# OmerMersin/video-stab

Measured on AMD Instinct MI355X. Metric: stabilized frames/sec @1080p (whole job; warp-stage HBM GB/s in roofline), higher is better.
Workload: dtype u8

## Files before the change

include/vs_stab.h:

```cpp
#ifndef VS_STAB_H
#define VS_STAB_H

#include <stddef.h>
#include <stdint.h>

#ifdef __cplusplus
extern "C" {
#endif

#define VS_STAB_ABI_VERSION 2

typedef enum vs_status {
    VS_OK = 0,
    VS_ERR_INVALID_ARG = 1,
    VS_ERR_NO_DEVICE = 2,
    VS_ERR_HIP = 3,
    VS_ERR_UNSUPPORTED = 4,
    VS_ERR_SIZE_CHANGED = 5,
    VS_ERR_CAPACITY = 6
} vs_status;

typedef enum vs_pixfmt {
    VS_FMT_BGR8 = 0,
    VS_FMT_NV12 = 1,
// ... 268 lines not shown
    int32_t push, idx, n_seen, has_M;
    float   M[12];
    double  Minv[12];
} vs_traj_release;
int vs_op_trajectory(const vs_params_c* params, int n_streams, const double* const* models, const int32_t* const* kinds,
                     const int32_t* n_push, int form, const int32_t* steps, int n_steps, vs_debug_frame* const* dbg_out,
                     int32_t* n_dbg, vs_traj_release* const* rel_out, int32_t* n_rel);
int vs_op_resize_gray(const void* d_src, size_t src_stride, int sw, int sh, int fmt,
                      void* d_dst, size_t dst_stride, int dw, int dh, void* stream);
int vs_op_pyr_down(const void* d_src, size_t src_stride, int sw, int sh,
                   void* d_dst, size_t dst_stride, void* stream);
int vs_op_scharr(const void* d_src, size_t src_stride, int w, int h,
                 void* d_dst , void* stream);
int vs_op_pyr_level(const void* d_src, size_t src_stride, size_t src_frame_bytes, int w, int h, void* d_der ,
                    void* d_next, size_t next_stride, size_t next_frame_bytes, int items, void* stream);
int vs_op_pyr_lk(const void* d_prev, const void* d_next, size_t stride, int w, int h,
                 const float* d_prev_pts, int n, float* d_next_pts,
                 uint8_t* d_status, float* d_err,
                 int win, int max_level, int max_iters, double eps, void* stream);
int vs_op_gftt(const void* d_gray, size_t stride, int w, int h, int max_corners,
               double quality, double min_distance, int block_size,
               float* d_pts, int32_t* d_count, float* d_eig, void* stream);
int vs_op_estimate_affine_partial2d(const float* d_from, const float* d_to, int n,
                                    double thr, int max_iters, double* d_model,
                                    uint8_t* d_inliers, int32_t* d_info, void* stream);

void vs_roll_params_default(vs_roll_params_c* p);
int vs_roll_create(const vs_roll_params_c* params, int device, vs_roll** out);
void vs_roll_destroy(vs_roll* r);
const char* vs_roll_last_error(const vs_roll* r);
// ... 140 lines not shown
```

video-stab_amd/csrc/batch_schedule.cpp:

```cpp
#include <cstring>
#include <new>

#include "stab_internal.h"

using namespace vsd;

struct vs_batch {
    int device = 0, S = 0, B = 0, cap = 0;
    bool own = false;
    std::vector<vs_stab*> m;
    vs_stab* ref = nullptr;
    std::string err;
    FirstFailure failure;
    hipStream_t st = nullptr, st_pre = nullptr, st_det = nullptr, st_up = nullptr;
    bool allocated = false;
    uint8_t* h_tables = nullptr;
    size_t h_set_bytes = 0, ho_pairs = 0, ho_lk = 0, ho_rs = 0, ho_tail = 0, ho_gf = 0, ho_seg = 0;
    uint8_t* d_all = nullptr;
    uint8_t *d_lk[2] = {nullptr, nullptr}, *d_rs[2] = {nullptr, nullptr}, *d_tail[2] = {nullptr, nullptr}, *d_seg[2] = {nullptr, nullptr}, *d_gf = nullptr;
    uint8_t* d_tin[2] = {nullptr, nullptr};
    ImgPair* d_pairs[2] = {nullptr, nullptr};
    size_t up_bytes = 0;
    int pre_rel_step = -1;
    double* d_MinvB[2] = {nullptr, nullptr};
// ... 304 lines not shown
    if (k >= 2) VS_OBJ_HIP(g, hipStreamWaitEvent(g->st_up, g->blk_event(k - 2), 0));
    VS_OBJ_HIP(g, hipMemcpyAsync(d_pairs, g->host_set(k).base, g->up_bytes, hipMemcpyHostToDevice, g->st_up));
    VS_OBJ_HIP(g, hipEventRecord(g->ev_up[dset], g->st_up));
    VS_OBJ_HIP(g, hipStreamWaitEvent(pre, g->ev_up[dset], 0));
    {
        StageScope t(g->ref, VS_STAGE_GRAY, pre);
        const int gfmt = s0->pf->gray_source;
        const int n_a = (P.ndet > 0 && P.ndet < n) ? P.ndet : n;
        VS_OBJ_TRY(g, launch_resize_gray_batch(d_pairs, n_a, s0->src_pitch, s0->w, s0->h, gfmt, s0->aw, s0->aw, s0->ah, P.aligned, pre));
        VS_OBJ_HIP(g, hipEventRecord(g->ev_bgray, pre));
        if (n_a < n)
            VS_OBJ_TRY(g, launch_resize_gray_batch(d_pairs + n_a, n - n_a, s0->src_pitch, s0->w, s0->h, gfmt, s0->aw, s0->aw, s0->ah, P.aligned, pre));
    }
    {
        StageScope t(g->ref, VS_STAGE_PYRAMID, pre);
        for (int l = 0; l < s0->levels; l++)
            VS_OBJ_TRY(g, launch_pyr_level_batch(nullptr, d_pairs + (size_t)(l + 1) * n, n, s0->lw[l], s0->lw[l], s0->lh[l], s0->lw[l + 1], pre));
    }
    if (!g->ready.valid) VS_OBJ_HIP(g, hipEventRecord(g->ev_bpre, pre));
    return VS_OK;
}

int step_issue_det(vs_batch* g, const StepPlan& P) {
    const vs_stab* s0 = g->ref;
    const int k = P.k, ndet = P.ndet;
    hipStream_t sd = g->st_det;
    g->det_valid(k) = ndet > 0;
    if (ndet == 0) return VS_OK;
    VS_OBJ_HIP(g, hipMemcpyAsync(g->d_gf, g->host_set(k).gf, gftt_item_bytes() * ndet, hipMemcpyHostToDevice, sd));
    if (k >= 2) VS_OBJ_HIP(g, hipStreamWaitEvent(sd, g->blk_event(k - 2), 0));
    VS_OBJ_TRY(g, launch_gftt_batch(g->d_gf, ndet, s0->aw, s0->ah, 3, sd, 1));
// ... 272 lines not shown
```

video-stab_amd/csrc/k_gftt.hip:

```cpp
#include <cstdio>
#include <cstdlib>

#include <cstring>

#include "vs_common.h"

namespace vsd {
namespace {

constexpr int TW = 64, TH = 16, NT = 256;
constexpr int MAX_BS = 7;

constexpr int SORT_CAP = 8192;
constexpr int CELLS_MAX = 2560;
constexpr int SLOTS = 4;
constexpr int ACC_MAX = 4096;
constexpr int SEL_NT = 256;
constexpr int NMS_ROWS = 8;

__device__ __forceinline__ uint32_t order_key(float v) {
    uint32_t b = __float_as_uint(v);
    return (b & 0x80000000u) ? ~b : (b | 0x80000000u);
}
__device__ __forceinline__ float key_to_float(uint32_t k) {
    uint32_t b = (k & 0x80000000u) ? (k & 0x7FFFFFFFu) : ~k;
    return __uint_as_float(b);
}

template <int BS>
__device__ __forceinline__ void min_eigen_tile(const uint8_t* __restrict__ gray, size_t stride, int w,
                                               int h, int bs_arg, float f1, float* __restrict__ eig,
                                               uint32_t* __restrict__ max_key) {
    constexpr int BSM = BS ? BS : MAX_BS;
    __shared__ uint8_t g[TH + BSM - 1 + 2][TW + BSM - 1 + 2 + 2];
    __shared__ float cxx[TH + BSM - 1][TW + BSM - 1 + 1], cxy[TH + BSM - 1][TW + BSM - 1 + 1], cyy[TH + BSM - 1][TW + BSM - 1 + 1];
    __shared__ uint32_t smax[NT / 64];
    const int bs = BS ? BS : bs_arg;
    const int tid = threadIdx.x;
    const int x0 = blockIdx.x * TW, y0 = blockIdx.y * TH;
    const int anchor = bs / 2, hi = bs - 1 - anchor;
    const int gx0 = x0 - anchor - 1, gy0 = y0 - anchor - 1;
    const int GW = TW + bs - 1 + 2, GH = TH + bs - 1 + 2;
    const int CW = TW + bs - 1, CH = TH + bs - 1;
    const float f0 = 2.f * f1;
    const bool interior = gx0 >= 0 && gy0 >= 0 && gx0 + GW <= w && gy0 + GH <= h;
    if (interior) {
        constexpr int NG = ((TW + BSM - 1 + 2) * (TH + BSM - 1 + 2) + NT - 1) / NT;
// ... 58 lines not shown
            const uint32_t k = order_key(e);
            kmax = k > kmax ? k : kmax;
        }
    }
#pragma unroll
    for (int off = 32; off >= 1; off >>= 1) {
        const uint32_t o = __shfl_xor(kmax, off, 64);
        kmax = o > kmax ? o : kmax;
    }
    if ((tid & 63) == 0) smax[tid >> 6] = kmax;
    __syncthreads();
    if (tid == 0) {
        uint32_t m = smax[0];
        for (int i = 1; i < NT / 64; i++) m = smax[i] > m ? smax[i] : m;
        atomicMax(max_key, m);
    }
}

template <int BS>
__global__ __launch_bounds__(NT) void min_eigen_kernel(const uint8_t* __restrict__ gray, size_t stride, int w,
                                                       int h, int bs, float f1, float* __restrict__ eig,
                                                       uint32_t* __restrict__ max_key) {
    min_eigen_tile<BS>(gray, stride, w, h, bs, f1, eig, max_key);
}

__device__ __forceinline__ void nms_row(const float* __restrict__ eig, int w, int h, double quality,
                                        const uint32_t* __restrict__ max_key,
                                        unsigned long long* __restrict__ cand, int cap,
                                        int32_t* __restrict__ counters) {
    const int x = blockIdx.x * blockDim.x + threadIdx.x;
    const float maxv = key_to_float(*max_key);
    const float thr = (float)((double)maxv * quality);
    const int lane = threadIdx.x & 63;
    float centre[NMS_ROWS];
    {
        const int xc = min(max(x, 0), w - 1);
#pragma unroll
        for (int k = 0; k < NMS_ROWS; k++) centre[k] = eig[(size_t)min((int)blockIdx.y * NMS_ROWS + k, h - 1) * w + xc];
    }
#pragma unroll
    for (int k = 0; k < NMS_ROWS; k++) {
    const int y = blockIdx.y * NMS_ROWS + k;
    if (y >= h) break;
    bool is_cand = false;
    float v = 0.f;
    if (x >= 1 && x < w - 1 && y >= 1 && y < h - 1) {
        const float* r = eig + (size_t)y * w + x;
        v = centre[k] > thr ? centre[k] : 0.f;
// ... 11 lines not shown
        }
    }
    const unsigned long long mask = __ballot(is_cand);
    if (!mask) continue;
    int base = 0;
    if (lane == __ffsll((long long)mask) - 1) base = atomicAdd(&counters[0], __popcll(mask));
    base = __builtin_amdgcn_readlane(base, __ffsll((long long)mask) - 1);
    if (!is_cand) continue;
    const int pos = base + __popcll(mask & ((1ull << lane) - 1ull));
    if (pos < cap) cand[pos] = ((unsigned long long)order_key(v) << 32) | (uint32_t)(y * w + x);
    else counters[2] = 1;
    }
}

__global__ __launch_bounds__(NT) void nms_kernel(const float* __restrict__ eig, int w, int h, double quality,
                                                 const uint32_t* __restrict__ max_key,
                                                 unsigned long long* __restrict__ cand, int cap,
                                                 int32_t* __restrict__ counters) {
    nms_row(eig, w, h, quality, max_key, cand, cap, counters);
}

struct SelArgs {
    const unsigned long long* cand;
    int32_t* counters;
    int cap, w, h, max_corners;
    int min_dist2_i;
    int use_dist;
    int cell, gw, gh;
    float* out_pts;
    int32_t* out_count;
};

template <int E>
__device__ __forceinline__ void bitonic_sort_desc(unsigned long long* keys, int tid) {
// ... 226 lines not shown
        a.counters[3] = s_nacc;
        if (s_overflow) a.counters[2] = 2;
    }
}

__global__ __launch_bounds__(SEL_NT) void select_kernel(SelArgs a) { select_corners(a); }

struct GfttItem {
    const uint8_t* gray;
    size_t stride;
    int w, h, bs;
    float f1;
    double quality;
    float* eig;
    int32_t* counters;
    SelArgs sel;
};

__global__ __launch_bounds__(64) void gftt_zero_batch_kernel(const GfttItem* __restrict__ table) {
    if (threadIdx.x < 16) table[blockIdx.x].counters[threadIdx.x] = 0;
}
template <int BS>
__global__ __launch_bounds__(NT) void min_eigen_batch_kernel(const GfttItem* __restrict__ table) {
    const GfttItem& it = table[blockIdx.z];
    min_eigen_tile<BS>(it.gray, it.stride, it.w, it.h, it.bs, it.f1, it.eig, (uint32_t*)&it.counters[1]);
}
__global__ __launch_bounds__(NT) void nms_batch_kernel(const GfttItem* __restrict__ table) {
    const GfttItem& it = table[blockIdx.z];
    nms_row(it.eig, it.w, it.h, it.quality, (const uint32_t*)&it.counters[1], (unsigned long long*)it.sel.cand, it.sel.cap,
            it.counters);
}
__global__ __launch_bounds__(SEL_NT) void select_batch_kernel(const GfttItem* __restrict__ table) {
    select_corners(table[blockIdx.x].sel);
}

bool gftt_bad_args(const uint8_t* d_gray, const float* d_pts, const int32_t* d_count, int w, int h, int max_corners,
                   int block_size, const GfttWork& wk) {
    return !d_gray || !d_pts || !d_count || w < 3 || h < 3 || w > 65535 || h > 65535 || max_corners <= 0 ||
           max_corners > ACC_MAX || block_size < 1 || block_size > MAX_BS || !wk.eig || !wk.cand || !wk.counters ||
           wk.cap <= 0;
}

void fill_sel_args(SelArgs& a, int w, int h, int max_corners, double min_distance, const GfttWork& wk, float* d_pts,
                   int32_t* d_count) {
    a.cand = (const unsigned long long*)wk.cand;
    a.counters = wk.counters;
    a.cap = wk.cap; a.w = w; a.h = h; a.max_corners = max_corners;
    a.use_dist = min_distance >= 1 ? 1 : 0;
    a.min_dist2_i = (int)std::ceil(std::min(min_distance * min_distance, 2.0e9));
    a.cell = a.use_dist ? (int)lrint(min_distance) : 1;
    a.gw = (w + a.cell - 1) / a.cell;
    a.gh = (h + a.cell - 1) / a.cell;
    a.out_pts = d_pts; a.out_count = d_count;
}
// ... 2 lines not shown

size_t gftt_item_bytes() { return sizeof(GfttItem); }

int gftt_fill_item(void* host_item, const uint8_t* d_gray, size_t stride, int w, int h, int max_corners, double quality,
                   double min_distance, int block_size, const GfttWork& wk, float* d_pts, int32_t* d_count) {
    if (!host_item || gftt_bad_args(d_gray, d_pts, d_count, w, h, max_corners, block_size, wk)) {
        set_last_error("gftt: invalid argument (1 <= blockSize <= 7, 0 < maxCorners <= 4096)");
        return VS_ERR_INVALID_ARG;
    }
    GfttItem& it = *static_cast<GfttItem*>(host_item);
    memset(&it, 0, sizeof it);
    it.gray = d_gray; it.stride = stride; it.w = w; it.h = h; it.bs = block_size;
    double scale = (double)(1 << 2) * block_size * 255.0;
    it.f1 = (float)(1.0 / scale);
    it.quality = quality;
    it.eig = wk.eig; it.counters = wk.counters;
    fill_sel_args(it.sel, w, h, max_corners, min_distance, wk, d_pts, d_count);
    return VS_OK;
}

int launch_gftt_batch(const void* d_table, int items, int w, int h, int block_size, hipStream_t st, int what) {
    if (!d_table || items < 1 || items > 65535 || w < 3 || h < 3 || block_size < 1 || block_size > MAX_BS || what < 0 || what > 5) { set_last_error("gftt_batch: invalid argument"); return VS_ERR_INVALID_ARG; }
    const GfttItem* t = static_cast<const GfttItem*>(d_table);
    if (what == 0 || what == 1) hipLaunchKernelGGL(gftt_zero_batch_kernel, dim3(items), dim3(64), 0, st, t);
    if (what == 0 || what == 2 || what == 4) {
        const dim3 eg((w + TW - 1) / TW, (h + TH - 1) / TH, items);
        if (block_size == 3) hipLaunchKernelGGL(min_eigen_batch_kernel<3>, eg, dim3(NT), 0, st, t);
        else hipLaunchKernelGGL(min_eigen_batch_kernel<0>, eg, dim3(NT), 0, st, t);
    }
    if (what == 0 || what == 2 || what == 5)
        hipLaunchKernelGGL(nms_batch_kernel, dim3((w + NT - 1) / NT, (h + NMS_ROWS - 1) / NMS_ROWS, items), dim3(NT), 0, st, t);
    if (what == 0 || what == 3) hipLaunchKernelGGL(select_batch_kernel, dim3(items), dim3(SEL_NT), 0, st, t);
    VS_HIP_TRY(hipGetLastError());
    return VS_OK;
}

size_t gftt_work_bytes(int w, int h, int cap) {
    return (size_t)w * h * 4 + (size_t)cap * 8 + 64 + 256;
}

void gftt_work_carve(void* base, int w, int h, int cap, GfttWork* out) {
    uint8_t* p = (uint8_t*)base;
    out->eig = (float*)p;
    p += ((size_t)w * h * 4 + 63) & ~(size_t)63;
    out->cand = (uint64_t*)p;
    p += (size_t)cap * 8;
    out->counters = (int32_t*)p;
    out->cap = cap;
}

int launch_gftt(const uint8_t* d_gray, size_t stride, int w, int h, int max_corners, double quality,
                double min_distance, int block_size, const GfttWork& wk, float* d_pts,
                int32_t* d_count, hipStream_t st) {
    if (gftt_bad_args(d_gray, d_pts, d_count, w, h, max_corners, block_size, wk)) {
        set_last_error("gftt: invalid argument (1 <= blockSize <= 7, 0 < maxCorners <= 4096)");
        return VS_ERR_INVALID_ARG;
    }
    VS_HIP_TRY(hipMemsetAsync(wk.counters, 0, 64, st));
    double scale = (double)(1 << 2) * block_size * 255.0;
    scale = 1.0 / scale;
    const float f1 = (float)scale;
    dim3 g1((w + TW - 1) / TW, (h + TH - 1) / TH);
    if (block_size == 3)
        hipLaunchKernelGGL(min_eigen_kernel<3>, g1, dim3(NT), 0, st, d_gray, stride, w, h, block_size, f1, wk.eig, (uint32_t*)&wk.counters[1]);
    else
        hipLaunchKernelGGL(min_eigen_kernel<0>, g1, dim3(NT), 0, st, d_gray, stride, w, h, block_size, f1, wk.eig, (uint32_t*)&wk.counters[1]);
    dim3 g2((w + NT - 1) / NT, (h + NMS_ROWS - 1) / NMS_ROWS);
    hipLaunchKernelGGL(nms_kernel, g2, dim3(NT), 0, st, wk.eig, w, h, quality, (const uint32_t*)&wk.counters[1],
                       (unsigned long long*)wk.cand, wk.cap, wk.counters);
    SelArgs a;
    fill_sel_args(a, w, h, max_corners, min_distance, wk, d_pts, d_count);
    hipLaunchKernelGGL(select_kernel, dim3(1), dim3(SEL_NT), 0, st, a);
    VS_HIP_TRY(hipGetLastError());
    return VS_OK;
}

int run_gftt_op(const uint8_t* d_gray, size_t stride, int w, int h, int max_corners, double quality,
                double min_distance, int block_size, float* d_pts, int32_t* d_count, float* d_eig,
                hipStream_t st) {
    if (w <= 0 || h <= 0) { set_last_error("gftt: invalid size"); return VS_ERR_INVALID_ARG; }
    const int cap = w * h / 4 + 64;
    void* scratch = nullptr;
    VS_HIP_TRY(hipMalloc(&scratch, gftt_work_bytes(w, h, cap)));
// ... 15 lines not shown
```

video-stab_amd/csrc/k_pyr.hip:

```cpp
#include "vs_common.h"

namespace vsd {
namespace {

constexpr int NT = 256;
constexpr int RPB = 4;

__global__ __launch_bounds__(NT) void pyr_down_kernel(const uint8_t* __restrict__ src_, size_t sstride,
                                                      int sw, int sh, uint8_t* __restrict__ dst_,
                                                      size_t dstride, int dw, int dh) {
    const uint8_t* __restrict__ src = src_;
    uint8_t* __restrict__ dst = dst_;
    const int x = blockIdx.x * blockDim.x + threadIdx.x;
    if (x >= dw) return;
    int xi[5];
#pragma unroll
    for (int k = 0; k < 5; k++) xi[k] = reflect101(2 * x + k - 2, sw);
    for (int y = blockIdx.y * RPB; y < min((int)(blockIdx.y + 1) * RPB, dh); y++) {
        int col[5];
#pragma unroll
        for (int j = 0; j < 5; j++) {
            const uint8_t* s = src + (size_t)reflect101(2 * y + j - 2, sh) * sstride;
            col[j] = s[xi[2]] * 6 + (s[xi[1]] + s[xi[3]]) * 4 + s[xi[0]] + s[xi[4]];
        }
// ... 17 lines not shown
    const int a_p = (r0[xp] + r2[xp]) * 3 + r1[xp] * 10;
    const int b_m = r2[xm] - r0[xm];
    const int b_c = r2[x] - r0[x];
    const int b_p = r2[xp] - r0[xp];
    short2 o;
    o.x = (short)(a_p - a_m);
    o.y = (short)((b_p + b_m) * 3 + b_c * 10);
    *reinterpret_cast<short2*>(dst + ((size_t)y * w + x) * 2) = o;
    }
}

constexpr int FT_W = 64, FT_H = 16;
constexpr int FT_PITCH = 72;
constexpr int FT_ROWS = FT_H + 4;

template <bool DER, bool DOWN>
__global__ __launch_bounds__(NT) void pyr_level_kernel(const ImgPair* __restrict__ sch, const ImgPair* __restrict__ pyr, size_t sstride,
                                                       int w, int h, size_t dstride, int dw, int dh) {
    static_assert(DER || DOWN, "a level launch produces something");
    __shared__ __attribute__((aligned(16))) uint8_t tile[FT_ROWS * FT_PITCH];
    const uint8_t* __restrict__ src = static_cast<const uint8_t*>((DER ? sch : pyr)[blockIdx.z].src);
    const int tid = threadIdx.x;
    const int x0 = blockIdx.x * FT_W, y0 = blockIdx.y * FT_H;
    const bool inside = x0 >= 4 && y0 >= 2 && x0 + FT_W + 4 <= w && y0 + FT_H + 2 <= h && (sstride & 3) == 0 && ((uintptr_t)src & 3) == 0;
    if (inside) {
        constexpr int ND = (FT_ROWS * (FT_PITCH / 4) + NT - 1) / NT;
        uint32_t v[ND];
#pragma unroll
        for (int k = 0; k < ND; k++) {
            const int i = min(tid + NT * k, FT_ROWS * (FT_PITCH / 4) - 1);
// ... 45 lines not shown
                const int dx = a[k + 2] - a[k], dy = (b[k + 2] + b[k]) * 3 + b[k + 1] * 10;
                o[k] = ((uint32_t)dx & 0xFFFFu) | ((uint32_t)dy << 16);
            }
            int16_t* d = der + ((size_t)y * w + x) * 2;
            if (x + 3 < w && (((uintptr_t)d) & 15) == 0) {
                *reinterpret_cast<uint4*>(d) = make_uint4(o[0], o[1], o[2], o[3]);
            } else {
                for (int k = 0; k < 4 && x + k < w; k++) reinterpret_cast<uint32_t*>(d)[k] = o[k];
            }
        }
    }
    if (DOWN) {
        uint8_t* __restrict__ dst = static_cast<uint8_t*>(pyr[blockIdx.z].dst);
        const int xo = (x0 >> 1) + (tid & 31), yo = (y0 >> 1) + (tid >> 5);
        if (xo < dw && yo < dh) {
            const int o = 2 * (tid & 31) + 2, sh = o & 3;
            const uint32_t* q = T + 2 * (tid >> 5) * (FT_PITCH / 4) + (o >> 2);
            int col[5];
#pragma unroll
            for (int j = 0; j < 5; j++) {
                const uint32_t lo = q[j * (FT_PITCH / 4)], hi = q[j * (FT_PITCH / 4) + 1];
                const uint32_t four = __builtin_amdgcn_alignbyte(hi, lo, sh);
                const uint32_t fifth = (hi >> (8 * sh)) & 255u;
                col[j] = (int)__builtin_amdgcn_udot4(four, 0x04060401u, fifth, false);
            }
            dst[(size_t)yo * dstride + xo] = (uint8_t)((col[2] * 6 + (col[1] + col[3]) * 4 + col[0] + col[4] + 128) >> 8);
        }
    }
}

}

int launch_pyr_level_batch(const ImgPair* d_scharr_pairs, const ImgPair* d_pyr_pairs, int items, size_t sstride, int w, int h,
                           size_t dstride, hipStream_t st) {
    if ((!d_scharr_pairs && !d_pyr_pairs) || items < 1 || items > 65535 || w <= 0 || h <= 0 || h > 65535) {
        set_last_error("pyr_level_batch: invalid argument");
        return VS_ERR_INVALID_ARG;
    }
    const int dw = (w + 1) / 2, dh = (h + 1) / 2;
    dim3 grid((w + FT_W - 1) / FT_W, (h + FT_H - 1) / FT_H, items);
    if (!d_scharr_pairs)
        hipLaunchKernelGGL((pyr_level_kernel<false, true>), grid, dim3(NT), 0, st, d_scharr_pairs, d_pyr_pairs, sstride, w, h, dstride, dw, dh);
    else if (d_pyr_pairs)
        hipLaunchKernelGGL((pyr_level_kernel<true, true>), grid, dim3(NT), 0, st, d_scharr_pairs, d_pyr_pairs, sstride, w, h, dstride, dw, dh);
    else hipLaunchKernelGGL((pyr_level_kernel<true, false>), grid, dim3(NT), 0, st, d_scharr_pairs, d_pyr_pairs, sstride, w, h, dstride, dw, dh);
    VS_HIP_TRY(hipGetLastError());
    return VS_OK;
}

int launch_pyr_down(const uint8_t* d_src, size_t sstride, int sw, int sh, uint8_t* d_dst,
                    size_t dstride, hipStream_t st) {
    if (!d_src || !d_dst || sw <= 0 || sh <= 0 || sh > 131070) {
        set_last_error("pyr_down: invalid argument");
        return VS_ERR_INVALID_ARG;
    }
    const int dw = (sw + 1) / 2, dh = (sh + 1) / 2;
    dim3 grid((dw + NT - 1) / NT, (dh + RPB - 1) / RPB);
    hipLaunchKernelGGL(pyr_down_kernel, grid, dim3(NT), 0, st, d_src, sstride, sw, sh, d_dst, dstride, dw, dh);
    VS_HIP_TRY(hipGetLastError());
    return VS_OK;
}

int launch_scharr(const uint8_t* d_src, size_t sstride, int w, int h, int16_t* d_dst, hipStream_t st) {
    if (!d_src || !d_dst || w <= 0 || h <= 0 || h > 65535) {
// ... 11 lines not shown
```

video-stab_amd/csrc/vs_api.cpp:

```cpp
#include <cmath>
#include <cstring>
#include <mutex>
#include <vector>

#include "launchers.h"
#include "vs_common.h"

namespace vsd {

static thread_local std::string g_last_error;
void set_last_error(const std::string& msg) { g_last_error = msg; }
const char* get_last_error() { return g_last_error.c_str(); }

int ensure_device() {
    int n = 0;
    hipError_t e = hipGetDeviceCount(&n);
    if (e != hipSuccess || n <= 0) {
        set_last_error(std::string("no HIP device: ") + (e != hipSuccess ? hipGetErrorString(e) : "count is 0") +
                       " (libvideo-stab has no CPU fallback)");
        return VS_ERR_NO_DEVICE;
    }
    return VS_OK;
}

// ... 305 lines not shown
        const uint8_t* s = (const uint8_t*)d_src + (size_t)i * src_frame_bytes;
        t[i] = ImgPair{s, (uint8_t*)d_der + (size_t)i * w * h * 4};
        t[items + i] = ImgPair{s, d_next ? (uint8_t*)d_next + (size_t)i * next_frame_bytes : nullptr};
    }
    ImgPair* d_t = nullptr;
    VS_HIP_TRY(hipMalloc((void**)&d_t, sizeof(ImgPair) * t.size()));
    hipStream_t st = (hipStream_t)stream;
    int rc = VS_OK;
    if (hipMemcpyAsync(d_t, t.data(), sizeof(ImgPair) * t.size(), hipMemcpyHostToDevice, st) != hipSuccess) rc = VS_ERR_HIP;
    if (rc == VS_OK) rc = launch_pyr_level_batch(d_t, d_next ? d_t + items : nullptr, items, src_stride, w, h, next_stride, st);
    (void)hipStreamSynchronize(st);
    (void)hipFree(d_t);
    return rc;
}

int vs_op_pyr_lk(const void* d_prev, const void* d_next, size_t stride, int w, int h,
                 const float* d_prev_pts, int n, float* d_next_pts, uint8_t* d_status, float* d_err,
                 int win, int max_level, int max_iters, double eps, void* stream) {
    VS_TRY(ensure_device());
    return run_pyr_lk_op((const uint8_t*)d_prev, (const uint8_t*)d_next, stride, w, h, d_prev_pts, n,
                         d_next_pts, d_status, d_err, win, max_level, max_iters, eps,
                         (hipStream_t)stream);
}

int vs_op_gftt(const void* d_gray, size_t stride, int w, int h, int max_corners, double quality,
               double min_distance, int block_size, float* d_pts, int32_t* d_count, float* d_eig,
               void* stream) {
    VS_TRY(ensure_device());
    return run_gftt_op((const uint8_t*)d_gray, stride, w, h, max_corners, quality, min_distance,
                       block_size, d_pts, d_count, d_eig, (hipStream_t)stream);
// ... 12 lines not shown
```

video-stab_amd/csrc/vs_common.h:

```cpp
#ifndef VS_COMMON_H
#define VS_COMMON_H

#include <hip/hip_runtime.h>
#include <cstdlib>
#include <stdint.h>
#include <cfloat>
#include <cmath>
#include <string>
#include <utility>

#include "../../include/vs_stab.h"

namespace vsd {

void set_last_error(const std::string& msg);
const char* get_last_error();

inline int hip_fail(hipError_t e, const char* expr) {
    set_last_error(std::string(expr) + ": " + hipGetErrorString(e));
    return (e == hipErrorNoDevice || e == hipErrorInvalidDevice || e == hipErrorInsufficientDriver || e == hipErrorNoBinaryForGpu)
               ? VS_ERR_NO_DEVICE
               : VS_ERR_HIP;
}

// ... 113 lines not shown
    int32_t sw, sh, dw, dh, cn, border;
    double m[6];
    int32_t sb = 1;
};
constexpr int WARP_JOBS_MAX = 24;
int launch_warp_jobs(const WarpJob* jobs, int n, hipStream_t st);
bool scale_job_staged(const WarpJob& j);
int launch_scale_jobs(const WarpJob* jobs, int n, int path, hipStream_t st);
int launch_resize_gray(const uint8_t* d_src, size_t sstride, int sw, int sh, int fmt,
                       uint8_t* d_dst, size_t dstride, int dw, int dh, hipStream_t st);
struct ImgPair { const void* src; void* dst; };
int launch_resize_gray_batch(const ImgPair* d_pairs, int items, size_t sstride, int sw, int sh, int fmt, size_t dstride,
                             int dw, int dh, int aligned, hipStream_t st);
int launch_pyr_level_batch(const ImgPair* d_scharr_pairs, const ImgPair* d_pyr_pairs, int items, size_t sstride, int w, int h,
                           size_t dstride, hipStream_t st);
int launch_pyr_down(const uint8_t* d_src, size_t sstride, int sw, int sh, uint8_t* d_dst,
                    size_t dstride, hipStream_t st);
int launch_scharr(const uint8_t* d_src, size_t sstride, int w, int h, int16_t* d_dst,
                  hipStream_t st);

struct LKLevel {
    const uint8_t* prev;
    const uint8_t* next;
    int w, h;
    size_t stride;
};
int launch_pyr_lk(const LKLevel* levels, int max_level, const float* d_prev_pts, int n,
                  const int32_t* d_n, float* d_next_pts, uint8_t* d_status, float* d_err, int win,
                  int max_iters, double eps, hipStream_t st);

struct GfttWork {
    float* eig;
    uint64_t* cand;
    int32_t* counters;
    int cap;
};
size_t gftt_work_bytes(int w, int h, int cap);
void gftt_work_carve(void* base, int w, int h, int cap, GfttWork* out);
int launch_gftt(const uint8_t* d_gray, size_t stride, int w, int h, int max_corners,
                double quality, double min_distance, int block_size, const GfttWork& wk,
                float* d_pts, int32_t* d_count, hipStream_t st);

}
#endif
```

video-stab_amd/vsamd/capi.py:

```python
import collections
import ctypes as C
import os

import numpy as np

PKG_DIR = os.path.dirname(os.path.dirname(os.path.abspath(__file__)))
LIB_PATH = os.path.join(PKG_DIR, "csrc", "libvideo-stab.so")

u8p = C.POINTER(C.c_uint8)
f32p = C.POINTER(C.c_float)
f64p = C.POINTER(C.c_double)
i32p = C.POINTER(C.c_int32)

PixFmt = collections.namedtuple("PixFmt", "fmt name text kind cn sample_bytes bits sx sy gray_source border_modes")
KIND_INTERLEAVED, KIND_LUMA_UV, KIND_THREE_PLANES = range(3)
PIXFMTS = (
    PixFmt(0, "BGR8", "BGR8", KIND_INTERLEAVED, 3, 1, 8, 0, 0, 0, True),
    PixFmt(1, "NV12", "NV12", KIND_LUMA_UV, 1, 1, 8, 1, 1, 2, False),
    PixFmt(2, "GRAY8", "GRAY8", KIND_INTERLEAVED, 1, 1, 8, 0, 0, 2, False),
    PixFmt(3, "BGRA8", "BGRA8", KIND_INTERLEAVED, 4, 1, 8, 0, 0, 3, True),
    PixFmt(4, "RGBA8", "RGBA8", KIND_INTERLEAVED, 4, 1, 8, 0, 0, 4, True),
    PixFmt(5, "RGB8", "RGB8", KIND_INTERLEAVED, 3, 1, 8, 0, 0, 5, True),
    PixFmt(6, "P010", "P010", KIND_LUMA_UV, 2, 2, 10, 1, 1, 6, False),
    PixFmt(7, "I420", "I420", KIND_THREE_PLANES, 1, 1, 8, 1, 1, 2, False),
# ... 311 lines not shown
                                       C.POINTER(C.c_int32), C.c_int, C.POINTER(C.c_int32), C.c_int, C.POINTER(C.POINTER(VsDebugFrame)),
                                       C.POINTER(C.c_int32), C.POINTER(C.POINTER(VsTrajRelease)), C.POINTER(C.c_int32)]
        L.vs_op_warp_affine.argtypes = [vp, C.c_size_t, C.c_size_t, vp, C.c_size_t, C.c_size_t, C.c_int, C.c_int,
                                        C.c_int, f32p, C.c_int, vp]
        L.vs_op_warp_affine_p010.argtypes = [vp, C.c_size_t, vp, C.c_size_t, C.c_int, C.c_int, f32p, C.c_int, C.c_size_t, C.c_size_t, vp]
        L.vs_op_warp_affine_nv12.argtypes = [vp, C.c_size_t, vp, C.c_size_t, C.c_int, C.c_int, f32p, C.c_int,
                                             C.c_size_t, C.c_size_t, vp]
        L.vs_op_warp_affine_i420.argtypes = [vp, C.c_size_t, C.c_size_t, C.c_size_t, C.c_size_t, vp, C.c_size_t, C.c_size_t, C.c_size_t, C.c_size_t,
                                             C.c_int, C.c_int, f32p, C.c_int, C.c_size_t, C.c_size_t, C.c_int, vp]
        L.vs_op_warp_affine_i010.argtypes = L.vs_op_warp_affine_i420.argtypes
        L.vs_op_warp_affine_planar.argtypes = [C.c_int] + list(L.vs_op_warp_affine_i420.argtypes)
        L.vs_op_resize_gray.argtypes = [vp, C.c_size_t, C.c_int, C.c_int, C.c_int, vp, C.c_size_t, C.c_int, C.c_int, vp]
        L.vs_op_pyr_down.argtypes = [vp, C.c_size_t, C.c_int, C.c_int, vp, C.c_size_t, vp]
        L.vs_op_scharr.argtypes = [vp, C.c_size_t, C.c_int, C.c_int, vp, vp]
        L.vs_op_pyr_level.argtypes = [vp, C.c_size_t, C.c_size_t, C.c_int, C.c_int, vp, vp, C.c_size_t, C.c_size_t, C.c_int, vp]
        L.vs_op_pyr_lk.argtypes = [vp, vp, C.c_size_t, C.c_int, C.c_int, vp, C.c_int, vp, vp, vp,
                                   C.c_int, C.c_int, C.c_int, C.c_double, vp]
        L.vs_op_gftt.argtypes = [vp, C.c_size_t, C.c_int, C.c_int, C.c_int, C.c_double, C.c_double, C.c_int,
                                 vp, vp, vp, vp]
        L.vs_op_estimate_affine_partial2d.argtypes = [vp, vp, C.c_int, C.c_double, C.c_int, vp, vp, vp, vp]
        L.vs_roll_params_default.argtypes = [C.POINTER(VsRollParams)]
        L.vs_roll_params_default.restype = None
        L.vs_roll_create.argtypes = [C.POINTER(VsRollParams), C.c_int, C.POINTER(vp)]
        L.vs_roll_destroy.argtypes = [vp]
        L.vs_roll_destroy.restype = None
        L.vs_roll_last_error.argtypes = [vp]
        L.vs_roll_last_error.restype = C.c_char_p
        L.vs_roll_correct.argtypes = [vp, u8p, C.c_int, C.c_int, C.c_size_t, u8p, C.c_size_t]
        L.vs_roll_correct_dev.argtypes = [vp, vp, C.c_int, C.c_int, C.c_size_t, vp, C.c_size_t]
        L.vs_roll_correct_nv12_dev.argtypes = [vp, vp, C.c_int, C.c_int, C.c_size_t, C.c_size_t, vp, C.c_size_t, C.c_size_t]
# ... 237 lines not shown
        self.check(self.lib.vs_op_scharr(d_in.ptr, w, w, h, d_out.ptr, None))
        self.sync()
        return d_out.download((h, w, 2), np.int16)

    def pyr_level(self, g, down=True):
        g = np.ascontiguousarray(g)
        h, w = g.shape
        dh, dw = (h + 1) // 2, (w + 1) // 2
        d_in = DevBuf.from_array(self, g)
        d_der = DevBuf(self, h * w * 4)
        d_next = DevBuf(self, dw * dh) if down else None
        self.check(self.lib.vs_op_pyr_level(d_in.ptr, w, w * h, w, h, d_der.ptr, d_next.ptr if down else None, dw, dw * dh, 1, None))
        self.sync()
        return d_der.download((h, w, 2), np.int16), (d_next.download((dh, dw), np.uint8) if down else None)

    def pyr_lk(self, prev, nxt, pts, win=15, max_level=2, iters=20, eps=0.03):
        prev = np.ascontiguousarray(prev)
        nxt = np.ascontiguousarray(nxt)
        pts = np.ascontiguousarray(pts, np.float32).reshape(-1, 2)
        n = pts.shape[0]
        h, w = prev.shape
        d_prev = DevBuf.from_array(self, prev)
        d_next = DevBuf.from_array(self, nxt)
        d_pts = DevBuf.from_array(self, pts)
        d_out = DevBuf(self, n * 8)
        d_st = DevBuf(self, n)
        d_err = DevBuf(self, n * 4)
        self.check(self.lib.vs_op_pyr_lk(d_prev.ptr, d_next.ptr, w, w, h, d_pts.ptr, n, d_out.ptr, d_st.ptr,
                                         d_err.ptr, win, max_level, iters, eps, None))
        self.sync()
# ... 837 lines not shown
```

Baseline: 128,600.

## Fuse two pyramid levels per kernel and skip GFTT NMS tiles below threshold

Adds a kernel that builds two pyramid downsample levels in one pass. It keeps the intermediate level in shared memory for the second downsample, which removes a launch and a global re-read of level 1. The GFTT min-eigen kernel now also records a per-tile maximum, and NMS exits early for tiles whose maximum cannot pass the quality threshold. The fused kernel adds complex halo and reflect-border logic that could differ from the two-pass output at edges.

```diff
diff --git a/include/vs_stab.h b/include/vs_stab.h
--- a/include/vs_stab.h
+++ b/include/vs_stab.h
@@ -306,6 +306,8 @@
                  void* d_dst , void* stream);
 int vs_op_pyr_level(const void* d_src, size_t src_stride, size_t src_frame_bytes, int w, int h, void* d_der ,
                     void* d_next, size_t next_stride, size_t next_frame_bytes, int items, void* stream);
+int vs_op_pyr_levels2(const void* d_src, size_t src_stride, size_t src_frame_bytes, int w, int h, void* d_l1, size_t l1_stride,
+                      size_t l1_frame_bytes, void* d_l2, size_t l2_stride, size_t l2_frame_bytes, int items, void* stream);
 int vs_op_pyr_lk(const void* d_prev, const void* d_next, size_t stride, int w, int h,
                  const float* d_prev_pts, int n, float* d_next_pts,
                  uint8_t* d_status, float* d_err,
diff --git a/video-stab_amd/csrc/batch_schedule.cpp b/video-stab_amd/csrc/batch_schedule.cpp
--- a/video-stab_amd/csrc/batch_schedule.cpp
+++ b/video-stab_amd/csrc/batch_schedule.cpp
@@ -342,7 +342,11 @@
     }
     {
         StageScope t(g->ref, VS_STAGE_PYRAMID, pre);
-        for (int l = 0; l < s0->levels; l++)
+        int l = 0;
+        for (; l + 2 <= s0->levels; l += 2)
+            VS_OBJ_TRY(g, launch_pyr_levels2_batch(d_pairs + (size_t)(l + 1) * n, d_pairs + (size_t)(l + 2) * n, n, s0->lw[l], s0->lw[l], s0->lh[l],
+                                                   s0->lw[l + 1], s0->lw[l + 2], pre));
+        if (l < s0->levels)
             VS_OBJ_TRY(g, launch_pyr_level_batch(nullptr, d_pairs + (size_t)(l + 1) * n, n, s0->lw[l], s0->lw[l], s0->lh[l], s0->lw[l + 1], pre));
     }
     if (!g->ready.valid) VS_OBJ_HIP(g, hipEventRecord(g->ev_bpre, pre));
diff --git a/video-stab_amd/csrc/k_gftt.hip b/video-stab_amd/csrc/k_gftt.hip
--- a/video-stab_amd/csrc/k_gftt.hip
+++ b/video-stab_amd/csrc/k_gftt.hip
@@ -30,7 +30,7 @@
 template <int BS>
 __device__ __forceinline__ void min_eigen_tile(const uint8_t* __restrict__ gray, size_t stride, int w,
                                                int h, int bs_arg, float f1, float* __restrict__ eig,
-                                               uint32_t* __restrict__ max_key) {
+                                               uint32_t* __restrict__ max_key, uint32_t* __restrict__ tile_max) {
     constexpr int BSM = BS ? BS : MAX_BS;
     __shared__ uint8_t g[TH + BSM - 1 + 2][TW + BSM - 1 + 2 + 2];
     __shared__ float cxx[TH + BSM - 1][TW + BSM - 1 + 1], cxy[TH + BSM - 1][TW + BSM - 1 + 1], cyy[TH + BSM - 1][TW + BSM - 1 + 1];
@@ -119,24 +119,31 @@
         uint32_t m = smax[0];
         for (int i = 1; i < NT / 64; i++) m = smax[i] > m ? smax[i] : m;
         atomicMax(max_key, m);
+        tile_max[blockIdx.y * gridDim.x + blockIdx.x] = m;
     }
 }
 
 template <int BS>
 __global__ __launch_bounds__(NT) void min_eigen_kernel(const uint8_t* __restrict__ gray, size_t stride, int w,
                                                        int h, int bs, float f1, float* __restrict__ eig,
-                                                       uint32_t* __restrict__ max_key) {
-    min_eigen_tile<BS>(gray, stride, w, h, bs, f1, eig, max_key);
+                                                       uint32_t* __restrict__ max_key, uint32_t* __restrict__ tile_max) {
+    min_eigen_tile<BS>(gray, stride, w, h, bs, f1, eig, max_key, tile_max);
 }
 
 __device__ __forceinline__ void nms_row(const float* __restrict__ eig, int w, int h, double quality,
-                                        const uint32_t* __restrict__ max_key,
+                                        const uint32_t* __restrict__ max_key, const uint32_t* __restrict__ tile_max,
                                         unsigned long long* __restrict__ cand, int cap,
                                         int32_t* __restrict__ counters) {
     const int x = blockIdx.x * blockDim.x + threadIdx.x;
     const float maxv = key_to_float(*max_key);
     const float thr = (float)((double)maxv * quality);
     const int lane = threadIdx.x & 63;
+    {
+        const int tx = __builtin_amdgcn_readfirstlane(x) / TW, ntx = (w + TW - 1) / TW;
+        if (tx >= ntx) return;
+        const uint32_t tkey = tile_max[(int)(blockIdx.y * NMS_ROWS / TH) * ntx + tx];
+        if (!(key_to_float(tkey) > thr)) return;
+    }
     float centre[NMS_ROWS];
     {
         const int xc = min(max(x, 0), w - 1);
@@ -178,10 +185,10 @@
 }
 
 __global__ __launch_bounds__(NT) void nms_kernel(const float* __restrict__ eig, int w, int h, double quality,
-                                                 const uint32_t* __restrict__ max_key,
+                                                 const uint32_t* __restrict__ max_key, const uint32_t* __restrict__ tile_max,
                                                  unsigned long long* __restrict__ cand, int cap,
                                                  int32_t* __restrict__ counters) {
-    nms_row(eig, w, h, quality, max_key, cand, cap, counters);
+    nms_row(eig, w, h, quality, max_key, tile_max, cand, cap, counters);
 }
 
 struct SelArgs {
@@ -438,6 +445,7 @@
     double quality;
     float* eig;
     int32_t* counters;
+    uint32_t* tile_max;
     SelArgs sel;
 };
 
@@ -447,11 +455,11 @@
 template <int BS>
 __global__ __launch_bounds__(NT) void min_eigen_batch_kernel(const GfttItem* __restrict__ table) {
     const GfttItem& it = table[blockIdx.z];
-    min_eigen_tile<BS>(it.gray, it.stride, it.w, it.h, it.bs, it.f1, it.eig, (uint32_t*)&it.counters[1]);
+    min_eigen_tile<BS>(it.gray, it.stride, it.w, it.h, it.bs, it.f1, it.eig, (uint32_t*)&it.counters[1], it.tile_max);
 }
 __global__ __launch_bounds__(NT) void nms_batch_kernel(const GfttItem* __restrict__ table) {
     const GfttItem& it = table[blockIdx.z];
-    nms_row(it.eig, it.w, it.h, it.quality, (const uint32_t*)&it.counters[1], (unsigned long long*)it.sel.cand, it.sel.cap,
+    nms_row(it.eig, it.w, it.h, it.quality, (const uint32_t*)&it.counters[1], it.tile_max, (unsigned long long*)it.sel.cand, it.sel.cap,
             it.counters);
 }
 __global__ __launch_bounds__(SEL_NT) void select_batch_kernel(const GfttItem* __restrict__ table) {
@@ -461,7 +469,7 @@
 bool gftt_bad_args(const uint8_t* d_gray, const float* d_pts, const int32_t* d_count, int w, int h, int max_corners,
                    int block_size, const GfttWork& wk) {
     return !d_gray || !d_pts || !d_count || w < 3 || h < 3 || w > 65535 || h > 65535 || max_corners <= 0 ||
-           max_corners > ACC_MAX || block_size < 1 || block_size > MAX_BS || !wk.eig || !wk.cand || !wk.counters ||
+           max_corners > ACC_MAX || block_size < 1 || block_size > MAX_BS || !wk.eig || !wk.cand || !wk.counters || !wk.tile_max ||
            wk.cap <= 0;
 }
 
@@ -494,7 +502,7 @@
     double scale = (double)(1 << 2) * block_size * 255.0;
     it.f1 = (float)(1.0 / scale);
     it.quality = quality;
-    it.eig = wk.eig; it.counters = wk.counters;
+    it.eig = wk.eig; it.counters = wk.counters; it.tile_max = wk.tile_max;
     fill_sel_args(it.sel, w, h, max_corners, min_distance, wk, d_pts, d_count);
     return VS_OK;
 }
@@ -515,8 +523,10 @@
     return VS_OK;
 }
 
+static size_t gftt_tiles(int w, int h) { return (size_t)((w + TW - 1) / TW) * ((h + TH - 1) / TH); }
+
 size_t gftt_work_bytes(int w, int h, int cap) {
-    return (size_t)w * h * 4 + (size_t)cap * 8 + 64 + 256;
+    return (size_t)w * h * 4 + (size_t)cap * 8 + 64 + 256 + gftt_tiles(w, h) * 4;
 }
 
 void gftt_work_carve(void* base, int w, int h, int cap, GfttWork* out) {
@@ -526,6 +536,8 @@
     out->cand = (uint64_t*)p;
     p += (size_t)cap * 8;
     out->counters = (int32_t*)p;
+    p += 64;
+    out->tile_max = (uint32_t*)p;
     out->cap = cap;
 }
 
@@ -542,11 +554,11 @@
     const float f1 = (float)scale;
     dim3 g1((w + TW - 1) / TW, (h + TH - 1) / TH);
     if (block_size == 3)
-        hipLaunchKernelGGL(min_eigen_kernel<3>, g1, dim3(NT), 0, st, d_gray, stride, w, h, block_size, f1, wk.eig, (uint32_t*)&wk.counters[1]);
+        hipLaunchKernelGGL(min_eigen_kernel<3>, g1, dim3(NT), 0, st, d_gray, stride, w, h, block_size, f1, wk.eig, (uint32_t*)&wk.counters[1], wk.tile_max);
     else
-        hipLaunchKernelGGL(min_eigen_kernel<0>, g1, dim3(NT), 0, st, d_gray, stride, w, h, block_size, f1, wk.eig, (uint32_t*)&wk.counters[1]);
+        hipLaunchKernelGGL(min_eigen_kernel<0>, g1, dim3(NT), 0, st, d_gray, stride, w, h, block_size, f1, wk.eig, (uint32_t*)&wk.counters[1], wk.tile_max);
     dim3 g2((w + NT - 1) / NT, (h + NMS_ROWS - 1) / NMS_ROWS);
-    hipLaunchKernelGGL(nms_kernel, g2, dim3(NT), 0, st, wk.eig, w, h, quality, (const uint32_t*)&wk.counters[1],
+    hipLaunchKernelGGL(nms_kernel, g2, dim3(NT), 0, st, wk.eig, w, h, quality, (const uint32_t*)&wk.counters[1], wk.tile_max,
                        (unsigned long long*)wk.cand, wk.cap, wk.counters);
     SelArgs a;
     fill_sel_args(a, w, h, max_corners, min_distance, wk, d_pts, d_count);
diff --git a/video-stab_amd/csrc/k_pyr.hip b/video-stab_amd/csrc/k_pyr.hip
--- a/video-stab_amd/csrc/k_pyr.hip
+++ b/video-stab_amd/csrc/k_pyr.hip
@@ -55,6 +55,24 @@
 constexpr int FT_PITCH = 72;
 constexpr int FT_ROWS = FT_H + 4;
 
+__device__ __forceinline__ int row_tap(const uint32_t* q, int sh) {
+    const uint32_t lo = q[0], hi = q[1];
+    const uint32_t four = __builtin_amdgcn_alignbyte(hi, lo, sh);
+    const uint32_t fifth = (hi >> (8 * sh)) & 255u;
+    return (int)__builtin_amdgcn_udot4(four, 0x04060401u, fifth, false);
+}
+__device__ __forceinline__ uint8_t col_tap(int c0, int c1, int c2, int c3, int c4) {
+    return (uint8_t)((c2 * 6 + (c1 + c3) * 4 + c0 + c4 + 128) >> 8);
+}
+__device__ __forceinline__ uint8_t down_tap(const uint32_t* q, int pitch4, int o) {
+    const int sh = o & 3;
+    q += o >> 2;
+    int col[5];
+#pragma unroll
+    for (int j = 0; j < 5; j++) col[j] = row_tap(q + j * pitch4, sh);
+    return col_tap(col[0], col[1], col[2], col[3], col[4]);
+}
+
 template <bool DER, bool DOWN>
 __global__ __launch_bounds__(NT) void pyr_level_kernel(const ImgPair* __restrict__ sch, const ImgPair* __restrict__ pyr, size_t sstride,
                                                        int w, int h, size_t dstride, int dw, int dh) {
@@ -130,18 +148,97 @@
         uint8_t* __restrict__ dst = static_cast<uint8_t*>(pyr[blockIdx.z].dst);
         const int xo = (x0 >> 1) + (tid & 31), yo = (y0 >> 1) + (tid >> 5);
         if (xo < dw && yo < dh) {
-            const int o = 2 * (tid & 31) + 2, sh = o & 3;
-            const uint32_t* q = T + 2 * (tid >> 5) * (FT_PITCH / 4) + (o >> 2);
-            int col[5];
-#pragma unroll
-            for (int j = 0; j < 5; j++) {
-                const uint32_t lo = q[j * (FT_PITCH / 4)], hi = q[j * (FT_PITCH / 4) + 1];
-                const uint32_t four = __builtin_amdgcn_alignbyte(hi, lo, sh);
-                const uint32_t fifth = (hi >> (8 * sh)) & 255u;
-                col[j] = (int)__builtin_amdgcn_udot4(four, 0x04060401u, fifth, false);
-            }
-            dst[(size_t)yo * dstride + xo] = (uint8_t)((col[2] * 6 + (col[1] + col[3]) * 4 + col[0] + col[4] + 128) >> 8);
-        }
+            const int o = 2 * (tid & 31) + 2;
+            dst[(size_t)yo * dstride + xo] = down_tap(T + 2 * (tid >> 5) * (FT_PITCH / 4), FT_PITCH / 4, o);
+        }
+    }
+}
+
+constexpr int F2_W = 128, F2_H = 32;
+constexpr int F2_PITCH = 144;
+constexpr int F2_ROWS = F2_H + 12;
+constexpr int F2_P4 = F2_PITCH / 4;
+constexpr int F2_NR = (F2_ROWS + 6) / 7;
+constexpr int F2_REG_W = FT_W + 4;
+
+__global__ __launch_bounds__(NT) void pyr_levels2_kernel(const ImgPair* __restrict__ p01, const ImgPair* __restrict__ p12, size_t sstride,
+                                                         int w, int h, size_t d1stride, int w1, int h1, size_t d2stride, int w2, int h2) {
+    __shared__ __attribute__((aligned(16))) uint8_t src0[F2_ROWS * F2_PITCH];
+    __shared__ __attribute__((aligned(16))) uint8_t tile[FT_ROWS * FT_PITCH];
+    const uint8_t* __restrict__ src = static_cast<const uint8_t*>(p01[blockIdx.z].src);
+    uint8_t* __restrict__ dst1 = static_cast<uint8_t*>(p01[blockIdx.z].dst);
+    uint8_t* __restrict__ dst2 = static_cast<uint8_t*>(p12[blockIdx.z].dst);
+    const int tid = threadIdx.x;
+    const int x0 = blockIdx.x * F2_W, y0 = blockIdx.y * F2_H;
+    if (tid < 7 * F2_P4) {
+        const int c4 = tid % F2_P4, r0 = tid / F2_P4;
+        const int xa = x0 - 8 + 4 * c4;
+        const bool aligned = (sstride & 3) == 0 && ((uintptr_t)src & 3) == 0;
+        const bool whole = aligned && xa >= 0 && xa + 3 < w;
+        size_t off[F2_NR];
+#pragma unroll
+        for (int k = 0; k < F2_NR; k++) off[k] = (size_t)reflect101(y0 - 6 + min(r0 + 7 * k, F2_ROWS - 1), h) * sstride;
+        uint32_t v[F2_NR];
+#pragma unroll
+        for (int k = 0; k < F2_NR; k++) v[k] = 0u;
+        if (whole) {
+            const uint8_t* col = src + xa;
+#pragma unroll
+            for (int k = 0; k < F2_NR; k++) v[k] = *reinterpret_cast<const uint32_t*>(col + off[k]);
+        } else if (xa <= w + 5) {
+            int cx[4];
+#pragma unroll
+            for (int b = 0; b < 4; b++) cx[b] = reflect101(xa + b, w);
+            uint8_t t[F2_NR][4];
+#pragma unroll
+            for (int k = 0; k < F2_NR; k++)
+#pragma unroll
+                for (int b = 0; b < 4; b++) t[k][b] = src[off[k] + cx[b]];
+#pragma unroll
+            for (int k = 0; k < F2_NR; k++) v[k] = (uint32_t)t[k][0] | ((uint32_t)t[k][1] << 8) | ((uint32_t)t[k][2] << 16) | ((uint32_t)t[k][3] << 24);
+        }
+#pragma unroll
+        for (int k = 0; k < F2_NR; k++)
+            if (r0 + 7 * k < F2_ROWS) reinterpret_cast<uint32_t*>(src0)[(r0 + 7 * k) * F2_P4 + c4] = v[k];
+    }
+    __syncthreads();
+    const uint32_t* S = reinterpret_cast<const uint32_t*>(src0);
+    const int x1_0 = x0 >> 1, y1_0 = y0 >> 1;
+    if (tid < 3 * F2_REG_W) {
+        const int strip = tid / F2_REG_W, j = tid - strip * F2_REG_W;
+        const int nrow = min(7, FT_ROWS - 7 * strip);
+        const int x1 = x1_0 - 2 + j, ya = y1_0 - 2 + 7 * strip;
+        const int cs = min(max(2 * reflect101(x1, w1) - 2 - (x0 - 8), 0), F2_PITCH - 8);
+        const uint32_t* q = S + (cs >> 2);
+        const int sh = cs & 3;
+        uint8_t val[7];
+        if (ya + nrow <= h1) {
+            int hs[17];
+#pragma unroll
+            for (int t = 0; t < 17; t++) hs[t] = row_tap(q + min(14 * strip + t, F2_ROWS - 1) * F2_P4, sh);
+#pragma unroll
+            for (int o = 0; o < 7; o++) val[o] = col_tap(hs[2 * o], hs[2 * o + 1], hs[2 * o + 2], hs[2 * o + 3], hs[2 * o + 4]);
+        } else {
+#pragma unroll
+            for (int o = 0; o < 7; o++) {
+                const int rs = min(max(2 * reflect101(ya + o, h1) - 2 - (y0 - 6), 0), F2_ROWS - 5);
+                val[o] = down_tap(S + rs * F2_P4, F2_P4, cs);
+            }
+        }
+#pragma unroll
+        for (int o = 0; o < 7; o++) {
+            const int r = 7 * strip + o, y1 = ya + o;
+            if (o < nrow) {
+                tile[r * FT_PITCH + j + 2] = val[o];
+                if (j >= 2 && j < 2 + FT_W && r >= 2 && r < 2 + FT_H && x1 < w1 && y1 < h1) dst1[(size_t)y1 * d1stride + x1] = val[o];
+            }
+        }
+    }
+    __syncthreads();
+    const int xo = (x1_0 >> 1) + (tid & 31), yo = (y1_0 >> 1) + (tid >> 5);
+    if (xo < w2 && yo < h2) {
+        const int o = 2 * (tid & 31) + 2;
+        dst2[(size_t)yo * d2stride + xo] = down_tap(reinterpret_cast<const uint32_t*>(tile) + 2 * (tid >> 5) * (FT_PITCH / 4), FT_PITCH / 4, o);
     }
 }
 
@@ -164,6 +261,23 @@
     return VS_OK;
 }
 
+int launch_pyr_levels2_batch(const ImgPair* d_pairs01, const ImgPair* d_pairs12, int items, size_t sstride, int w, int h, size_t d1stride,
+                             size_t d2stride, hipStream_t st) {
+    if (!d_pairs01 || !d_pairs12 || items < 1 || items > 65535 || w <= 0 || h <= 0 || h > 65535) {
+        set_last_error("pyr_levels2_batch: invalid argument");
+        return VS_ERR_INVALID_ARG;
+    }
+    const int w1 = (w + 1) / 2, h1 = (h + 1) / 2, w2 = (w1 + 1) / 2, h2 = (h1 + 1) / 2;
+    if (w < 8 || h < 8) {
+        VS_TRY(launch_pyr_level_batch(nullptr, d_pairs01, items, sstride, w, h, d1stride, st));
+        return launch_pyr_level_batch(nullptr, d_pairs12, items, d1stride, w1, h1, d2stride, st);
+    }
+    dim3 grid((w + F2_W - 1) / F2_W, (h + F2_H - 1) / F2_H, items);
+    hipLaunchKernelGGL(pyr_levels2_kernel, grid, dim3(NT), 0, st, d_pairs01, d_pairs12, sstride, w, h, d1stride, w1, h1, d2stride, w2, h2);
+    VS_HIP_TRY(hipGetLastError());
+    return VS_OK;
+}
+
 int launch_pyr_down(const uint8_t* d_src, size_t sstride, int sw, int sh, uint8_t* d_dst,
                     size_t dstride, hipStream_t st) {
     if (!d_src || !d_dst || sw <= 0 || sh <= 0 || sh > 131070) {
diff --git a/video-stab_amd/csrc/vs_api.cpp b/video-stab_amd/csrc/vs_api.cpp
--- a/video-stab_amd/csrc/vs_api.cpp
+++ b/video-stab_amd/csrc/vs_api.cpp
@@ -343,6 +343,27 @@
     return rc;
 }
 
+int vs_op_pyr_levels2(const void* d_src, size_t src_stride, size_t src_frame_bytes, int w, int h, void* d_l1, size_t l1_stride, size_t l1_frame_bytes,
+                      void* d_l2, size_t l2_stride, size_t l2_frame_bytes, int items, void* stream) {
+    VS_TRY(ensure_device());
+    if (!d_src || !d_l1 || !d_l2 || items < 1 || items > 4096 || w <= 0 || h <= 0) { set_last_error("pyr_levels2: invalid argument"); return VS_ERR_INVALID_ARG; }
+    std::vector<ImgPair> t(2 * (size_t)items);
+    for (int i = 0; i < items; i++) {
+        uint8_t* l1 = (uint8_t*)d_l1 + (size_t)i * l1_frame_bytes;
+        t[i] = ImgPair{(const uint8_t*)d_src + (size_t)i * src_frame_bytes, l1};
+        t[items + i] = ImgPair{l1, (uint8_t*)d_l2 + (size_t)i * l2_frame_bytes};
+    }
+    ImgPair* d_t = nullptr;
+    VS_HIP_TRY(hipMalloc((void**)&d_t, sizeof(ImgPair) * t.size()));
+    hipStream_t st = (hipStream_t)stream;
+    int rc = VS_OK;
+    if (hipMemcpyAsync(d_t, t.data(), sizeof(ImgPair) * t.size(), hipMemcpyHostToDevice, st) != hipSuccess) rc = VS_ERR_HIP;
+    if (rc == VS_OK) rc = launch_pyr_levels2_batch(d_t, d_t + items, items, src_stride, w, h, l1_stride, l2_stride, st);
+    (void)hipStreamSynchronize(st);
+    (void)hipFree(d_t);
+    return rc;
+}
+
 int vs_op_pyr_lk(const void* d_prev, const void* d_next, size_t stride, int w, int h,
                  const float* d_prev_pts, int n, float* d_next_pts, uint8_t* d_status, float* d_err,
                  int win, int max_level, int max_iters, double eps, void* stream) {
diff --git a/video-stab_amd/csrc/vs_common.h b/video-stab_amd/csrc/vs_common.h
--- a/video-stab_amd/csrc/vs_common.h
+++ b/video-stab_amd/csrc/vs_common.h
@@ -151,6 +151,8 @@
                              int dw, int dh, int aligned, hipStream_t st);
 int launch_pyr_level_batch(const ImgPair* d_scharr_pairs, const ImgPair* d_pyr_pairs, int items, size_t sstride, int w, int h,
                            size_t dstride, hipStream_t st);
+int launch_pyr_levels2_batch(const ImgPair* d_pairs01, const ImgPair* d_pairs12, int items, size_t sstride, int w, int h, size_t d1stride,
+                             size_t d2stride, hipStream_t st);
 int launch_pyr_down(const uint8_t* d_src, size_t sstride, int sw, int sh, uint8_t* d_dst,
                     size_t dstride, hipStream_t st);
 int launch_scharr(const uint8_t* d_src, size_t sstride, int w, int h, int16_t* d_dst,
@@ -170,6 +172,7 @@
     float* eig;
     uint64_t* cand;
     int32_t* counters;
+    uint32_t* tile_max;
     int cap;
 };
 size_t gftt_work_bytes(int w, int h, int cap);
diff --git a/video-stab_amd/vsamd/capi.py b/video-stab_amd/vsamd/capi.py
--- a/video-stab_amd/vsamd/capi.py
+++ b/video-stab_amd/vsamd/capi.py
@@ -349,6 +349,7 @@
         L.vs_op_pyr_down.argtypes = [vp, C.c_size_t, C.c_int, C.c_int, vp, C.c_size_t, vp]
         L.vs_op_scharr.argtypes = [vp, C.c_size_t, C.c_int, C.c_int, vp, vp]
         L.vs_op_pyr_level.argtypes = [vp, C.c_size_t, C.c_size_t, C.c_int, C.c_int, vp, vp, C.c_size_t, C.c_size_t, C.c_int, vp]
+        L.vs_op_pyr_levels2.argtypes = [vp, C.c_size_t, C.c_size_t, C.c_int, C.c_int, vp, C.c_size_t, C.c_size_t, vp, C.c_size_t, C.c_size_t, C.c_int, vp]
         L.vs_op_pyr_lk.argtypes = [vp, vp, C.c_size_t, C.c_int, C.c_int, vp, C.c_int, vp, vp, vp,
                                    C.c_int, C.c_int, C.c_int, C.c_double, vp]
         L.vs_op_gftt.argtypes = [vp, C.c_size_t, C.c_int, C.c_int, C.c_int, C.c_double, C.c_double, C.c_int,
@@ -616,6 +617,22 @@
         self.sync()
         return d_der.download((h, w, 2), np.int16), (d_next.download((dh, dw), np.uint8) if down else None)
 
+    def pyr_levels2(self, imgs, pitch=None):
+        imgs = np.ascontiguousarray(imgs, np.uint8)
+        n, h, w = imgs.shape
+        pitch = pitch or w
+        h1, w1, h2, w2 = (h + 1) // 2, (w + 1) // 2, ((h + 1) // 2 + 1) // 2, ((w + 1) // 2 + 1) // 2
+        padded = np.zeros((n, h, pitch), np.uint8)
+        padded[:, :, :w] = imgs
+        d_in = DevBuf.from_array(self, padded)
+        d_l1, d_l2 = DevBuf(self, n * w1 * h1), DevBuf(self, n * w2 * h2)
+        try:
+            self.check(self.lib.vs_op_pyr_levels2(d_in.ptr, pitch, pitch * h, w, h, d_l1.ptr, w1, w1 * h1, d_l2.ptr, w2, w2 * h2, n, None))
+            self.sync()
+            return d_l1.download((n, h1, w1), np.uint8), d_l2.download((n, h2, w2), np.uint8)
+        finally:
+            d_in.free(); d_l1.free(); d_l2.free()
+
     def pyr_lk(self, prev, nxt, pts, win=15, max_level=2, iters=20, eps=0.03):
         prev = np.ascontiguousarray(prev)
         nxt = np.ascontiguousarray(nxt)
```

Result: no change. 130,200, median of 2 (+1.2%).
